# Artessay/RAGraph

Measured on AMD Instinct MI355X. Metric: retrieved-queries/sec (RAGraph_node forward: GCN encode + cosine/top-k retrieval + 3-hop propagate + decode), higher is better.
Workload: dtype f32 (exact results; candidates pre-filtered on bf16 / int8 MFMA with proven bounds)

## Files before the change

include/ragraph_hip.h:

```cpp
#ifndef RAGRAPH_HIP_H
#define RAGRAPH_HIP_H

#include <stddef.h>
#include <stdint.h>

#ifdef __cplusplus
extern "C" {
#endif

#define RAGRAPH_ABI_VERSION 1

#define RAGRAPH_OK 0
#define RAGRAPH_EINVAL (-1)
#define RAGRAPH_EUNSUPPORTED (-2)
#define RAGRAPH_EWORKSPACE (-3)
#define RAGRAPH_EDEVICE (-4)

#define RAGRAPH_ACT_NONE 0
#define RAGRAPH_ACT_RELU 1
#define RAGRAPH_ACT_PRELU 2
#define RAGRAPH_ACT_LEAKY 3
#define RAGRAPH_ACT_ELU 4

int ragraph_abi_version(void);
// ... 148 lines not shown
                               const int64_t* off, int64_t E, int64_t* out_col, int64_t* out_r, float* out_val,
                               void* stream);
int ragraph_spmm_csr_prelu_dev_f32(const int64_t* rowptr, const int32_t* col, const float* val, int64_t n, const float* X,
                                   int D, const float* bias, const float* alpha, float* Y, float* Z, int64_t nnz, void* ws,
                                   size_t ws_bytes, void* stream);
int ragraph_act_grad_prelu_dev_f32(const float* z, const float* gy, int64_t n, const float* alpha, float* gz,
                                   float* alpha_terms, void* stream);

size_t ragraph_radix_sort_workspace_bytes(int64_t n, int val_bytes);
int ragraph_radix_sort_u64(const uint64_t* keys_in, uint64_t* keys_out, const void* vals_in, void* vals_out, int val_bytes,
                           int64_t n, int bits, void* ws, size_t ws_bytes, void* stream);
size_t ragraph_scan_workspace_bytes(int64_t n);
int ragraph_scan_sum_i32(const int* in, int* out, int64_t n, int inclusive, void* ws, size_t ws_bytes, void* stream);

size_t ragraph_coo_to_csr_workspace_bytes(int64_t E, int64_t n);
int ragraph_coo_to_csr_i64(const int64_t* row, const int64_t* col, int64_t E, int64_t n, int sort_cols, int64_t* rowptr,
                           int64_t* perm, int32_t* out_col, void* ws, size_t ws_bytes, void* stream);
int ragraph_csr_row_ids_i64(const int64_t* rowptr, int64_t n, int64_t nnz, int64_t* rows, void* stream);

size_t ragraph_dense_to_csr_workspace_bytes(int64_t rows, int64_t cols);
int ragraph_dense_to_csr_f32(const float* a, int64_t rows, int64_t cols, int64_t lda, int64_t capacity, int64_t* rowptr,
                             int32_t* col, float* val, int64_t* status, void* ws, size_t ws_bytes, void* stream);

size_t ragraph_mask_positions_workspace_bytes(int64_t E);
int ragraph_mask_positions_i64(const unsigned char* mask, int64_t E, int64_t* pos, int64_t* count, void* ws, size_t ws_bytes,
                               void* stream);

int ragraph_spmm_csr_panels_f32(const int64_t* rowptr, const int32_t* col, const float* val, int64_t n, const float* X,
                                int64_t x_rows, int x_panels, int D, int act, float alpha, float* Y, int y_panels, void* stream);

int ragraph_spmm_linear_f32(const int64_t* rowptr, const int32_t* col, const float* val, int64_t M, const float* X, int K,
                            const float* W, int64_t N, const float* bias, int act, float alpha, float* Y, void* stream);

int ragraph_spmm_csr_tiled_f32(const int* wp, const int* col3, const float* val3, const unsigned short* row3, int RG, int C,
                               int64_t n, const float* X, int64_t x_rows, int x_panels, int D, int act, float alpha, float* Y,
                               int y_panels, void* stream);

int ragraph_csr_row_normalize_f32(const int64_t* rowptr, const float* val, int64_t n, float* val_out, void* stream);

int ragraph_segment_softmax_f32(const int64_t* rowptr, const float* x, int64_t n, float* out, void* stream);
int ragraph_segment_softmax_ws_f32(const int64_t* rowptr, const float* x, int64_t n, int64_t nnz, float* out, void* ws,
                                   size_t ws_bytes, void* stream);

int ragraph_axpby_f32(const float* a, float wa, const float* b, float wb, int64_t n, float* out, void* stream);

#define RAGRAPH_INTERP_MAX_TABLES 8
int ragraph_interp_normalize_f32(const float* const* tables, const float* weights, int S, int64_t n, int D, float* out,
                                 void* stream);

int ragraph_fuse_decode_f32(const float* query, const float* rag, int64_t n, int D, float wq, float wr, const float* W1,
                            const float* b1, int H, float slope, const float* W2, const float* b2, int C,
                            const float* rag_label, float lambda, float* out, void* stream);

int ragraph_softmax_mix_f32(const float* logits, const float* rag_label, int64_t B, int C, float lambda, int log_mode,
                            float* out, void* stream);

int ragraph_segment_reduce_f32(const float* X, int D, const int64_t* seg_ptr, int64_t G, const float* w, int mean_mode,
                               float* out, void* stream);

int ragraph_proto_cosine_f32(const float* emb, int64_t G, int D, const float* proto, int C, int mode, float* out,
                             void* stream);

int ragraph_sigmoid_gate_f32(const float* x, const float* z, int64_t n, float* out, void* stream);

int ragraph_time_rescale_f32(const int64_t* t, int64_t n, float t_min, float t_max, float* out, void* stream);

int ragraph_topk_rows_f32(const float* S, int64_t B, int64_t N, int64_t ld, int k, float* out_scores,
                          int64_t* out_idx, void* stream);

int ragraph_topk_select_rows_f32(const float* S, int64_t B, int64_t N, int64_t ld, int64_t k, float* out_kth,
                                 int64_t* out_idx, void* stream);
size_t ragraph_topk_select_rows_workspace_bytes(int64_t B, int64_t N);
int ragraph_topk_select_rows_ws_f32(const float* S, int64_t B, int64_t N, int64_t ld, int64_t k, float* out_kth,
                                    int64_t* out_idx, void* ws, size_t ws_bytes, void* stream);

#define RAGRAPH_TOPK_ORDERED_MAX 4096
size_t ragraph_topk_rows_large_workspace_bytes(int64_t B, int64_t N, int64_t k);
int ragraph_topk_rows_large_f32(const float* S, int64_t B, int64_t N, int64_t ld, int64_t k, float* out_scores,
                                int64_t* out_idx, void* ws, size_t ws_bytes, void* stream);

int ragraph_scatter_fill_f32(float* S, int64_t B, int64_t N, int64_t ld, const int64_t* rowptr, const int64_t* col,
                             float value, void* stream);

int ragraph_floyd_warshall_f32(const float* adj, int n, float* dist, void* stream);

int ragraph_position_code_f32(const float* dist, int n, const int64_t* anchors, int A, float dis_q, float* out,
                              void* stream);

int ragraph_position_codes_csr_f32(const int64_t* rowptr, const int32_t* col, const float* val, int64_t n,
                                   const int64_t* anchors, int A, float dis_q, float* codes, float* dist, void* stream);

#define RAGRAPH_POSITION_CODES_LONG_ROW 512
size_t ragraph_position_codes_csr_global_workspace_bytes(int64_t n, int A);
int ragraph_position_codes_csr_global_f32(const int64_t* rowptr, const int32_t* col, const float* val, int64_t n,
                                          const int64_t* anchors, int A, float dis_q, float* codes, float* dist, int rounds,
                                          int resume, int32_t* converged, void* ws, size_t ws_bytes, void* stream);

int ragraph_act_grad_f32(const float* y, const float* gy, int64_t n, int act, float alpha, float* gz, float* alpha_terms,
                         void* stream);
int ragraph_sigmoid_gate_grad_f32(const float* x, const float* z, const float* g, int64_t n, float* gx, float* gz, void* stream);
int ragraph_softmax_grad_f32(const float* p, const float* go, int64_t B, int C, float scale, float* out, void* stream);
int ragraph_mul_cols_f32(const float* x, const float* w, int64_t n, int D, float* out, void* stream);
int ragraph_mul_cols_act_f32(const float* x, const float* w, int64_t n, int D, int act, float alpha, float* out, void* stream);
int ragraph_mul_f32(const float* a, const float* b, int64_t n, float* out, void* stream);
int ragraph_proto_cosine_grad_f32(const float* emb, int64_t G, int D, const float* proto, int C, int mode, const float* out,
                                  const float* gout, float* gemb, void* stream);
// ... 79 lines not shown
```

ragraph_amd/RAGraph.py:

```python
import functools
import os

import torch
import torch.nn as nn

from . import autograd as A
from . import kernels as K
from .graph import as_csr
from .ragraph_utils import Propagation, TaskDecoder, ToyGraphBase


class RAGraph(nn.Module):

    flavour = "node"

    def __init__(self, pretrain_model, resource_dataset, feture_size, num_class, emb_size, finetune=True,
                 noise_finetune=False, device="cuda", build_rng="host") -> None:
        super().__init__()
        self.emb_size = emb_size
        self.num_class = num_class
        self.pretrain_model = pretrain_model
        self.retrieve_weight, self.label_weight, self.query_graph_hop = self._hyper()
        self.finetune = finetune
        self.noise_finetune = noise_finetune
# ... 9 lines not shown
            self.reset_parameters()
        self.to(device)

    def _hyper(self):
        return 0.5, 0.5, 3

    def reset_parameters(self):
        self.decoder.reset_parameters()

    def _queries(self, emb, g):
        return emb

    def _pool(self, x, g):
        return x

    query_shard = None

    def forward(self, features, adj, anchors=None):
        g = as_csr(adj)
        tgb = self.toy_graph_base
        mixed = getattr(tgb, "structure_weight", 0.0) != 0
        if mixed and (self.query_shard is not None or hasattr(tgb, "retrieve_reduced_rows")):
            raise K.RagraphNativeError("structure-aware retrieval (structure_weight != 0) runs on one GPU with the whole "
                                       "bank: the query-sharded and key-sharded forwards do not mix position codes")
        shards_queries = self.query_shard is not None and not self.training and self.flavour == "node"
        own_rows = not self.training and self.flavour == "node" and self._finishes_own_rows(tgb)
        if shards_queries:
            sliced = self._forward_sliced_encode(features, g, hybrid=own_rows)
            if sliced is not None:
                return sliced
        pretrain_embedddings = self.pretrain_model.inference(features, g)
        add_noise = self.training and self.noise_finetune
        if add_noise and getattr(tgb, "noise_rng", "host") != "device" and torch.cuda.is_current_stream_capturing():
            raise K.RagraphNativeError("noisy fine-tuning draws its noise on the host generator, as the reference does: "
                                       "its step cannot be captured in a HIP graph (train it eagerly, or set "
                                       "toy_graph_base.noise_rng = 'device')")
        queries = self._queries(pretrain_embedddings, g)
        pos = tgb.search_positions(g, None, anchors) if mixed else None
        if own_rows:
            return self._forward_key_shard(queries, pretrain_embedddings, g)
        if shards_queries:
            return self._forward_query_shard(queries, pretrain_embedddings, g)
        def hops():
            return self._pool(Propagation.aggregate_k_hop_features(g, pretrain_embedddings, self.query_graph_hop), g)

        join = None
        if (self.finetune and not (torch.is_grad_enabled() and pretrain_embedddings.requires_grad) and queries.is_cuda
                and queries.shape[0] >= self.OVERLAP_MIN_NODES):
            join = self._fork(hops, queries.device)
        if (join is not None and not add_noise and not torch.is_grad_enabled() and self.flavour == "node"
                and type(tgb).retrieve_reduced is ToyGraphBase.retrieve_reduced
                and os.environ.get("RAGRAPH_GATHER_MIX", "1") != "0"):
            _, idx = tgb.topk(queries, tgb.retrieve_num, pos) if mixed else tgb.topk(queries, tgb.retrieve_num)
            hidden, rag_label = K.gather_reduce_mix(tgb.resource_values, tgb.resource_labels, idx, join(),
                                                    1 - self.retrieve_weight, self.retrieve_weight)
            return A.softmax_mix(self.decoder(hidden), rag_label, self.label_weight)
        if add_noise:
            rag_embedding, rag_label = (tgb.retrieve_reduced_noisy(queries, search_positions=pos) if mixed
                                        else tgb.retrieve_reduced_noisy(queries))
        elif mixed:
            rag_embedding, rag_label, _ = tgb.retrieve_reduced(queries, search_positions=pos)
        else:
            rag_embedding, rag_label, _ = tgb.retrieve_reduced(queries)
        if not self.finetune:
            return rag_label
        query_embeddings = join() if join is not None else hops()
        return self._fuse_decode(query_embeddings, rag_embedding, rag_label)

    OVERLAP_MIN_NODES = 16384

    @staticmethod
    def _finishes_own_rows(tgb) -> bool:
        return (getattr(tgb, "values_replicated", False) and hasattr(tgb, "retrieve_reduced_rows")
                and (tgb.collective or tgb.emulate_world > 1))

    def _side_stream(self, device):
        st = getattr(self, "_side", None)
        if st is None or st.device != device:
            st = torch.cuda.Stream(device=device)
            self._side = st
        return st

    def _fork(self, fn, device):
        main = torch.cuda.current_stream()
        side = self._side_stream(device)
        side.wait_stream(main)
        with torch.cuda.stream(side):
            out = fn()

        def join():
            main.wait_stream(side)
            out.record_stream(main)
            return out
        return join

    def _fuse_decode(self, query_embeddings, rag_embedding, rag_label):
        fc1, fc2 = self.decoder.layers()
        trains = torch.is_grad_enabled() and (query_embeddings.requires_grad or rag_embedding.requires_grad or
                                              any(p.requires_grad for p in self.decoder.parameters()))
        if not trains and K.fuse_decode_fits(query_embeddings.shape[0], fc1.in_features, fc1.out_features, fc2.out_features):
            return K.fuse_decode(query_embeddings, rag_embedding, 1 - self.retrieve_weight, self.retrieve_weight,
                                 fc1.weight, fc1.bias, self.decoder.NEGATIVE_SLOPE, fc2.weight, fc2.bias, rag_label,
                                 self.label_weight)
        hidden = A.axpby(query_embeddings, 1 - self.retrieve_weight, rag_embedding, self.retrieve_weight)
        decode_label = self.decoder(hidden)
        return A.softmax_mix(decode_label, rag_label, self.label_weight)
# ... 79 lines not shown
```

ragraph_amd/_native.py:

```python
from __future__ import annotations

import ctypes
import os
import subprocess

import torch

_HERE = os.path.dirname(os.path.abspath(__file__))
CSRC = os.path.join(_HERE, "csrc")
SO_PATH = os.environ.get("RAGRAPH_HIP_SO", os.path.join(CSRC, "libragraph_hip.so"))

OK, EINVAL, EUNSUPPORTED, EWORKSPACE, EDEVICE = 0, -1, -2, -3, -4
ACT_NONE, ACT_RELU, ACT_PRELU, ACT_LEAKY, ACT_ELU = 0, 1, 2, 3, 4
TOPK_MAX = 64
TOPK_FILTER_MAX = 128
TOPK_ORDERED_MAX = 4096
TOPK_TAIL_MAX = 65536
LINEAR_GENERIC, LINEAR_SMALL, LINEAR_TILE, LINEAR_STREAM, LINEAR_NARROW = 0, 1, 2, 3, 4
INTERP_MAX_TABLES = 8
POSITION_CODES_LDS_MAX = 40000
POSITION_CODES_LONG_ROW = 512

_vp, _i64, _i32, _f32, _sz = ctypes.c_void_p, ctypes.c_int64, ctypes.c_int, ctypes.c_float, ctypes.c_size_t

# ... 49 lines not shown
    "ragraph_topk_cosine_mix_workspace_bytes": (_sz, [_i64, _i64, _i32, _i32, _i32]),
    "ragraph_topk_cosine_mix_f32": (_i32, [_vp, _i64, _vp, _i64, _i32, _vp, _vp, _i32, _f32, _f32, _i32, _i64, _vp, _vp, _vp,
                                          _sz, _vp]),
    "ragraph_topk_mix_rerank_workspace_bytes": (_sz, [_i64, _i32]),
    "ragraph_topk_mix_rerank_f32": (_i32, [_vp, _vp, _i64, _i32, _vp, _vp, _i64, _i32, _f32, _f32, _i32, _i64, _vp, _vp, _vp, _vp,
                                          _vp, _sz, _vp]),
    "ragraph_topk_rows_scatter_f32": (_i32, [_vp, _vp, _vp, _i64, _i32, _i64, _vp, _vp, _vp]),
    "ragraph_topk_merge_f32": (_i32, [_vp, _vp, _i32, _i64, _i32, _vp, _vp, _vp]),
    "ragraph_topk_cosine_tail_workspace_bytes": (_sz, [_i64, _i64, _i32, _i32]),
    "ragraph_topk_cosine_tail_f32": (_i32, [_vp, _i64, _vp, _i64, _i32, _i32, _i64, _vp, _vp, _vp, _vp, _vp, _sz, _vp]),
    "ragraph_topk_drop_rows_f32": (_i32, [_vp, _vp, _i64, _i32, _i64, _vp, _i64, _i32, _vp, _vp, _vp, _vp]),
    "ragraph_rows_retire_u32": (_i32, [_vp, _i64, _i64, _vp, _vp]),
    "ragraph_dedup_rows_workspace_bytes": (_sz, [_i64]),
    "ragraph_dedup_rows_f32": (_i32, [_vp, _i64, _i32, _vp, _vp, _vp, _vp, _vp, _sz, _vp]),
    "ragraph_topk_expand_groups_f32": (_i32, [_vp, _vp, _i32, _i64, _vp, _vp, _i64, _i64, _i32, _i64, _vp, _vp, _vp]),
    "ragraph_gather_rows_f32": (_i32, [_vp, _i64, _i32, _vp, _i64, _i64, _vp, _vp]),
    "ragraph_gather_reduce_f32": (_i32, [_vp, _i32, _vp, _i32, _i64, _vp, _i64, _i32, _i64, _f32, _vp, _vp, _vp]),
    "ragraph_gather_reduce_mix_f32": (_i32, [_vp, _i32, _vp, _i32, _i64, _vp, _i64, _i32, _i64, _f32, _vp, _f32, _f32, _vp, _vp, _vp]),
    "ragraph_linear_f32": (_i32, [_vp, _i64, _i32, _vp, _i64, _vp, _i32, _f32, _vp, _vp]),
    "ragraph_linear_plan": (_i32, [_i64, _i32, _i64, _i32, _i32, _vp]),
    "ragraph_linear_tn_workspace_bytes": (_sz, [_i64, _i32, _i32]),
    "ragraph_linear_tn_f32": (_i32, [_vp, _vp, _i64, _i32, _i32, _vp, _vp, _sz, _vp]),
    "ragraph_spmm_csr_f32": (_i32, [_vp, _vp, _vp, _i64, _vp, _i32, _vp, _i32, _f32, _f32, _vp, _vp, _vp]),
    "ragraph_radix_sort_workspace_bytes": (_sz, [_i64, _i32]),
    "ragraph_radix_sort_u64": (_i32, [_vp, _vp, _vp, _vp, _i32, _i64, _i32, _vp, _sz, _vp]),
    "ragraph_scan_workspace_bytes": (_sz, [_i64]),
    "ragraph_scan_sum_i32": (_i32, [_vp, _vp, _i64, _i32, _vp, _sz, _vp]),
    "ragraph_coo_to_csr_workspace_bytes": (_sz, [_i64, _i64]),
    "ragraph_coo_to_csr_i64": (_i32, [_vp, _vp, _i64, _i64, _i32, _vp, _vp, _vp, _vp, _sz, _vp]),
    "ragraph_csr_row_ids_i64": (_i32, [_vp, _i64, _i64, _vp, _vp]),
    "ragraph_dense_to_csr_workspace_bytes": (_sz, [_i64, _i64]),
    "ragraph_dense_to_csr_f32": (_i32, [_vp, _i64, _i64, _i64, _i64, _vp, _vp, _vp, _vp, _vp, _sz, _vp]),
    "ragraph_mask_positions_workspace_bytes": (_sz, [_i64]),
    "ragraph_mask_positions_i64": (_i32, [_vp, _i64, _vp, _vp, _vp, _sz, _vp]),
    "ragraph_spmm_csr_panels_f32": (_i32, [_vp, _vp, _vp, _i64, _vp, _i64, _i32, _i32, _i32, _f32, _vp, _i32, _vp]),
    "ragraph_spmm_linear_f32": (_i32, [_vp, _vp, _vp, _i64, _vp, _i32, _vp, _i64, _vp, _i32, _f32, _vp, _vp]),
    "ragraph_spmm_csr_tiled_f32": (_i32, [_vp, _vp, _vp, _vp, _i32, _i32, _i64, _vp, _i64, _i32, _i32, _i32, _f32, _vp, _i32, _vp]),
    "ragraph_csr_row_normalize_f32": (_i32, [_vp, _vp, _i64, _vp, _vp]),
    "ragraph_segment_softmax_f32": (_i32, [_vp, _vp, _i64, _vp, _vp]),
    "ragraph_segment_softmax_ws_f32": (_i32, [_vp, _vp, _i64, _i64, _vp, _vp, _sz, _vp]),
    "ragraph_sparse_workspace_bytes": (_sz, [_i64, _i32]),
    "ragraph_spmm_csr_ws_f32": (_i32, [_vp, _vp, _vp, _i64, _vp, _i32, _vp, _i32, _f32, _f32, _vp, _vp, _i64, _vp, _sz,
                                       _vp]),
    "ragraph_spmm_csr_rows_workspace_bytes": (_sz, [_i64, _i64, _i32]),
    "ragraph_spmm_csr_rows_f32": (_i32, [_vp, _vp, _vp, _i64, _vp, _i32, _vp, _i64, _vp, _i64, _vp, _sz, _vp]),
    "ragraph_csr_rows_offsets_workspace_bytes": (_sz, [_i64]),
    "ragraph_csr_rows_offsets_i64": (_i32, [_vp, _i64, _vp, _i64, _vp, _vp, _sz, _vp]),
    "ragraph_csr_rows_edges_f32": (_i32, [_vp, _vp, _vp, _vp, _i64, _vp, _i64, _vp, _vp, _vp, _vp]),
    "ragraph_axpby_f32": (_i32, [_vp, _f32, _vp, _f32, _i64, _vp, _vp]),
    "ragraph_interp_normalize_f32": (_i32, [_vp, _vp, _i32, _i64, _i32, _vp, _vp]),
    "ragraph_softmax_mix_f32": (_i32, [_vp, _vp, _i64, _i32, _f32, _i32, _vp, _vp]),
    "ragraph_fuse_decode_f32": (_i32, [_vp, _vp, _i64, _i32, _f32, _f32, _vp, _vp, _i32, _f32, _vp, _vp, _i32, _vp, _f32,
                                       _vp, _vp]),
    "ragraph_segment_reduce_f32": (_i32, [_vp, _i32, _vp, _i64, _vp, _i32, _vp, _vp]),
    "ragraph_proto_cosine_f32": (_i32, [_vp, _i64, _i32, _vp, _i32, _i32, _vp, _vp]),
    "ragraph_sigmoid_gate_f32": (_i32, [_vp, _vp, _i64, _vp, _vp]),
    "ragraph_time_rescale_f32": (_i32, [_vp, _i64, _f32, _f32, _vp, _vp]),
    "ragraph_topk_rows_f32": (_i32, [_vp, _i64, _i64, _i64, _i32, _vp, _vp, _vp]),
    "ragraph_topk_select_rows_f32": (_i32, [_vp, _i64, _i64, _i64, _i64, _vp, _vp, _vp]),
    "ragraph_topk_select_rows_workspace_bytes": (_sz, [_i64, _i64]),
    "ragraph_topk_select_rows_ws_f32": (_i32, [_vp, _i64, _i64, _i64, _i64, _vp, _vp, _vp, _sz, _vp]),
    "ragraph_topk_rows_large_workspace_bytes": (_sz, [_i64, _i64, _i64]),
    "ragraph_topk_rows_large_f32": (_i32, [_vp, _i64, _i64, _i64, _i64, _vp, _vp, _vp, _sz, _vp]),
    "ragraph_scatter_fill_f32": (_i32, [_vp, _i64, _i64, _i64, _vp, _vp, _f32, _vp]),
    "ragraph_floyd_warshall_f32": (_i32, [_vp, _i32, _vp, _vp]),
    "ragraph_position_code_f32": (_i32, [_vp, _i32, _vp, _i32, _f32, _vp, _vp]),
    "ragraph_position_codes_csr_f32": (_i32, [_vp, _vp, _vp, _i64, _vp, _i32, _f32, _vp, _vp, _vp]),
    "ragraph_position_codes_csr_global_workspace_bytes": (_sz, [_i64, _i32]),
    "ragraph_position_codes_csr_global_f32": (_i32, [_vp, _vp, _vp, _i64, _vp, _i32, _f32, _vp, _vp, _i32, _i32, _vp, _vp, _sz,
                                                     _vp]),
    "ragraph_act_grad_f32": (_i32, [_vp, _vp, _i64, _i32, _f32, _vp, _vp, _vp]),
    "ragraph_spmm_csr_prelu_dev_f32": (_i32, [_vp, _vp, _vp, _i64, _vp, _i32, _vp, _vp, _vp, _vp, _i64, _vp, _sz, _vp]),
    "ragraph_act_grad_prelu_dev_f32": (_i32, [_vp, _vp, _i64, _vp, _vp, _vp, _vp]),
    "ragraph_sigmoid_gate_grad_f32": (_i32, [_vp, _vp, _vp, _i64, _vp, _vp, _vp]),
    "ragraph_softmax_grad_f32": (_i32, [_vp, _vp, _i64, _i32, _f32, _vp, _vp]),
    "ragraph_mul_cols_f32": (_i32, [_vp, _vp, _i64, _i32, _vp, _vp]),
    "ragraph_mul_cols_act_f32": (_i32, [_vp, _vp, _i64, _i32, _i32, _f32, _vp, _vp]),
    "ragraph_mul_f32": (_i32, [_vp, _vp, _i64, _vp, _vp]),
    "ragraph_proto_cosine_grad_f32": (_i32, [_vp, _i64, _i32, _vp, _i32, _i32, _vp, _vp, _vp, _vp]),
    "ragraph_proto_cosine_grad_proto_workspace_bytes": (_sz, [_i64, _i32, _i32]),
    "ragraph_proto_cosine_grad_proto_f32": (_i32, [_vp, _i64, _i32, _vp, _i32, _i32, _vp, _vp, _vp, _vp, _sz, _vp]),
    "ragraph_axpby_dev_f32": (_i32, [_vp, _vp, _vp, _i32, _i32, _i64, _vp, _vp]),
    "ragraph_ingest_workspace_bytes": (_sz, [_i64, _i64]),
    "ragraph_csr_sym_normalized_f32": (_i32, [_vp, _vp, _i64, _i64, _vp, _vp, _vp, _vp, _vp, _sz, _vp]),
    "ragraph_binorm_edges_f32": (_i32, [_vp, _vp, _vp, _i64, _i64, _i64, _vp, _vp, _vp, _vp, _vp, _sz, _vp]),
    "ragraph_pagerank_workspace_bytes": (_sz, [_i64, _i64]),
    "ragraph_pagerank_f32": (_i32, [_vp, _vp, _vp, _vp, _vp, _vp, _i64, _i64, _f32, _f32, _i32, _vp, _vp, _vp, _sz, _vp]),
    "ragraph_sample_prob_f32": (_i32, [_vp, _vp, _vp, _i64, _f32, _f32, _vp, _vp]),
    "ragraph_csr_row_sums_f32": (_i32, [_vp, _vp, _i64, _vp, _vp]),
    "ragraph_position_codes_batch_f32": (_i32, [_vp, _i64, _i32, _vp, _i32, _f32, _vp, _vp, _vp]),
    "ragraph_topk_dot_masked_workspace_bytes": (_sz, [_i64, _i64, _i32, _i32, _i64]),
    "ragraph_topk_dot_masked_f32": (_i32, [_vp, _i64, _vp, _i64, _vp, _i64, _i32, _i32, _vp, _vp, _i64, _f32, _vp, _vp, _vp,
                                          _sz, _vp]),
    "ragraph_rank_metrics_workspace_bytes": (_sz, [_i64, _i32, _i64]),
    "ragraph_rank_metrics_f64": (_i32, [_vp, _i64, _i32, _vp, _vp, _vp, _i32, _i64, _vp, _vp, _sz, _vp]),
    "ragraph_lp_workspace_bytes": (_sz, []),
    "ragraph_lp_sample_i64": (_i32, [_vp, _vp, _i64, _i64, _i32, _vp, _vp, _vp, _sz, _vp]),
    "ragraph_lp_compare_loss_fwd_f32": (_i32, [_vp, _i64, _i32, _vp, _i32, _f32, _vp, _vp, _vp, _vp, _vp, _vp, _vp, _sz, _vp]),
    "ragraph_lp_combine_f32": (_i32, [_vp, _vp, _vp, _vp, _vp, _f32, _i64, _i32, _vp, _vp]),
    "ragraph_edge_hist_check_i64": (_i32, [_vp, _vp, _i64, _i64, _i64, _vp, _sz, _vp]),
    "ragraph_edge_neg_sample_i64": (_i32, [_vp, _vp, _i64, _i64, _vp, _i64, _i32, _i32, _vp, _vp, _vp, _sz, _vp]),
    "ragraph_noise_rows_i64": (_i32, [_vp, _vp, _i64, _i64, _i32, _i64, _vp, _i64, _vp]),
    "ragraph_gather_reduce_noisy_f32": (_i32, [_vp, _i32, _vp, _i32, _i64, _vp, _i64, _i32, _i64, _f32, _vp, _vp, _i64, _i32, _i64,
                                               _vp, _f32, _f32, _vp, _vp, _vp]),
    "ragraph_add_normal_noise_f32": (_i32, [_vp, _i64, _i64, _i32, _f32, _vp, _vp, _i64, _vp, _vp]),
    "ragraph_edge_rewrite_workspace_bytes": (_sz, [_i64]),
# ... 57 lines not shown
```

ragraph_amd/csrc/dense.hip:

```cpp
#include "common.h"

namespace ragraph {

constexpr int LBM = 64, LBN = 64, LKC = 32, LLD = LKC + 1;

__global__ void __launch_bounds__(256) linear_kernel(const float* __restrict__ X, int64_t M, int K,
                                                     const float* __restrict__ W, int64_t N,
                                                     const float* __restrict__ bias, int act, float alpha,
                                                     float* __restrict__ Y) {
  __shared__ float As[2][LBM * LLD];
  __shared__ float Bs[2][LBN * LLD];
  const int tid = threadIdx.x, lane = tid & 63, wave = tid >> 6;
  const int j = lane & 31, h = lane >> 5;
  const int wr = wave >> 1, wc = wave & 1;
  const int64_t m0 = (int64_t)blockIdx.x * LBM;
  const int64_t n0 = (int64_t)blockIdx.y * LBN;

  f32x16 acc;
#pragma unroll
  for (int r = 0; r < 16; ++r) acc[r] = 0.f;

  constexpr int PER = (LBM * LKC) / 256;
  float ra[2][PER], rb[2][PER];
  auto gload = [&](int k0, float (&pa)[PER], float (&pb)[PER]) {
#pragma unroll
    for (int u = 0; u < PER; ++u) {
      const int e = tid + u * 256;
      const int row = e / LKC, c = e % LKC;
      const int kk = k0 + c;
      const int64_t gm = m0 + row, gn = n0 + row;
      pa[u] = (gm < M && kk < K) ? X[gm * K + kk] : 0.f;
      pb[u] = (gn < N && kk < K) ? W[gn * K + kk] : 0.f;
    }
  };
  auto sstore = [&](int buf, const float (&pa)[PER], const float (&pb)[PER]) {
#pragma unroll
    for (int u = 0; u < PER; ++u) {
      const int e = tid + u * 256;
      const int row = e / LKC, c = e % LKC;
      As[buf][row * LLD + c] = pa[u];
      Bs[buf][row * LLD + c] = pb[u];
    }
  };
  auto compute = [&](int buf) {
    const float* a = As[buf] + (wr * 32 + j) * LLD + h;
    const float* b = Bs[buf] + (wc * 32 + j) * LLD + h;
#pragma unroll
    for (int kk = 0; kk < LKC / 2; ++kk) acc = __builtin_amdgcn_mfma_f32_32x32x2f32(a[2 * kk], b[2 * kk], acc, 0, 0, 0);
  };
  const int nch = (K + LKC - 1) / LKC;
  gload(0, ra[0], rb[0]);
  sstore(0, ra[0], rb[0]);
  if (nch > 1) gload(LKC, ra[1], rb[1]);
// ... 322 lines not shown
  for (int s = 0; s < nstages; ++s) {
    const bool more = s + 1 < nstages;
    stage_load(more ? s + 1 : s);
    __builtin_amdgcn_sched_barrier(0);
#pragma unroll 1
    for (int t = 0; t < C::TILES; ++t) {
      f32x16 acc;
#pragma unroll
      for (int r = 0; r < 16; ++r) acc[r] = 0.f;
      const float* arow = smem + (s & 1) * C::STAGE_FLOATS + (t * 32 + j) * C::ROW + h * (KD / 2);
#pragma unroll
      for (int c = 0; c < KD / 8; ++c) {
        const float4 v = *reinterpret_cast<const float4*>(arow + 4 * c);
        acc = __builtin_amdgcn_mfma_f32_32x32x2f32(v.x, breg[4 * c], acc, 0, 0, 0);
        acc = __builtin_amdgcn_mfma_f32_32x32x2f32(v.y, breg[4 * c + 1], acc, 0, 0, 0);
        acc = __builtin_amdgcn_mfma_f32_32x32x2f32(v.z, breg[4 * c + 2], acc, 0, 0, 0);
        acc = __builtin_amdgcn_mfma_f32_32x32x2f32(v.w, breg[4 * c + 3], acc, 0, 0, 0);
      }
      const int64_t m_base = (st0 + s) * C::STAGE_ROWS + t * 32 + 4 * h;
      if (n < N) {
#pragma unroll
        for (int r = 0; r < 16; ++r) {
          const int64_t m = m_base + (r & 3) + 8 * (r >> 2);
          if (m < M) {
            float v = acc[r];
            if (bias) v = __fadd_rn(v, bv);
            Y[m * N + n] = apply_act(v, act, alpha);
          }
        }
      }
    }
    if (more) stage_write((s + 1) & 1);
    __syncthreads();
  }
}

template <int KD>
struct AggLinCfg {
  static constexpr int THREADS = 1024, MFMA_THREADS = 512;
  static constexpr int LPR = KD / 4;
  static constexpr int GROUPS = (THREADS - MFMA_THREADS) / LPR;
  static constexpr int R = 2;
  static constexpr int STAGE_ROWS = R * GROUPS;
  static constexpr int TILES = STAGE_ROWS / 32;
  static constexpr int ROW = KD + 4;
  static constexpr int STAGE_FLOATS = STAGE_ROWS * ROW;
#ifndef RG_AGGLIN_NB
#define RG_AGGLIN_NB 4
#endif
  static constexpr int NB = RG_AGGLIN_NB;
  static constexpr size_t LDS_BYTES = sizeof(float) * NB * STAGE_FLOATS + sizeof(int) * 2 * NB;
};

__device__ __forceinline__ void agglin_wait(int* f, int target) {
#ifdef RG_AGGLIN_FREE_RUN
  return;
#endif
  int spins = 0;
  while (__hip_atomic_load(f, __ATOMIC_ACQUIRE, __HIP_MEMORY_SCOPE_WORKGROUP) < target) {
    __builtin_amdgcn_s_sleep(1);
    if (++spins > (1 << 26)) __builtin_trap();
  }
}
__device__ __forceinline__ void agglin_signal(int* f, int lane) {
  if (lane == 0) __hip_atomic_fetch_add(f, 1, __ATOMIC_RELEASE, __HIP_MEMORY_SCOPE_WORKGROUP);
}

template <int KD>
__global__ void __launch_bounds__(1024, 1) spmm_linear_stream_kernel(const int64_t* __restrict__ rowptr, const int32_t* __restrict__ col,
                                                                     const float* __restrict__ val, const float* __restrict__ X,
                                                                     int64_t M, const float* __restrict__ W, int64_t N,
                                                                     const float* __restrict__ bias, int act, float alpha,
                                                                     float* __restrict__ Y) {
  using C = AggLinCfg<KD>;
  extern __shared__ float4 lin_smem4[];
  float* smem = reinterpret_cast<float*>(lin_smem4);
  const int tid = threadIdx.x, lane = tid & 63, wave = __builtin_amdgcn_readfirstlane(tid >> 6);
  const int64_t total_stages = (M + C::STAGE_ROWS - 1) / C::STAGE_ROWS;
  const int64_t st0 = (int64_t)blockIdx.x * total_stages / gridDim.x;
  const int64_t st1 = (int64_t)(blockIdx.x + 1) * total_stages / gridDim.x;
  if (st0 >= st1) return;
  const int nstages = (int)(st1 - st0);
  int* ready = reinterpret_cast<int*>(smem + C::NB * C::STAGE_FLOATS);
  int* freed = ready + C::NB;
  if (tid < 2 * C::NB) ready[tid] = 0;
  __syncthreads();

  if (wave < 8) {
    const int j = lane & 31, h = lane >> 5;
    const int64_t n = (int64_t)blockIdx.y * 256 + wave * 32 + j;
    float breg[KD / 2];
    {
      const float4* wp = reinterpret_cast<const float4*>(W + (n < N ? n : N - 1) * KD);
#pragma unroll
      for (int c0 = 0; c0 < KD / 4; c0 += 16) {
#pragma unroll
        for (int c = c0; c < c0 + 16 && c < KD / 4; ++c) {
          const float4 v = wp[c];
          breg[2 * c] = h ? v.y : v.x;
          breg[2 * c + 1] = h ? v.w : v.z;
        }
#pragma unroll
        for (int c = c0; c < c0 + 16 && c < KD / 4; ++c) asm volatile("" : "+v"(breg[2 * c]), "+v"(breg[2 * c + 1]));
        asm volatile("" ::: "memory");
      }
    }
    const float bv = (bias && n < N) ? bias[n] : 0.f;
    for (int s = 0; s < nstages; ++s) {
      const int buf = s % C::NB;
      agglin_wait(ready + buf, 8 * (s / C::NB + 1));
#ifndef RG_AGGLIN_NO_MFMA
#pragma unroll 1
      for (int t = 0; t < C::TILES; ++t) {
        f32x16 acc;
#pragma unroll
        for (int r = 0; r < 16; ++r) acc[r] = 0.f;
        const float* arow = smem + buf * C::STAGE_FLOATS + (t * 32 + j) * C::ROW + h * (KD / 2);
#pragma unroll
        for (int c = 0; c < KD / 8; ++c) {
// ... 437 lines not shown
```

ragraph_amd/kernels.py:

```python
from __future__ import annotations

import collections
import ctypes
import os

import torch

from . import _native as N
from ._native import ACT_ELU, ACT_LEAKY, ACT_NONE, ACT_PRELU, ACT_RELU, RagraphNativeError
from ._native import LINEAR_GENERIC, LINEAR_NARROW, LINEAR_SMALL, LINEAR_STREAM, LINEAR_TILE
from .filter_stats import MAGIC_VALUE as FILTER_STATS_MAGIC, levels as filter_stats_levels, ord2f

_device_ok = False


def _ready():
    global _device_ok
    if not _device_ok:
        N.require_device()
        _device_ok = True
    return N.lib()


def _f32c(t: torch.Tensor, name: str) -> torch.Tensor:
# ... 929 lines not shown
        out = torch.empty_like(tables[0])
    elif (not isinstance(out, torch.Tensor) or out.dtype != torch.float32 or out.shape != tables[0].shape
          or out.device != tables[0].device or not out.is_contiguous()):
        raise RagraphNativeError("interp_normalize: out must be a contiguous fp32 tensor of the tables' shape and device")
    if n == 0:
        return out
    ptrs = (ctypes.c_void_p * len(tables))(*[t.data_ptr() for t in tables])
    ws = (ctypes.c_float * len(w))(*w)
    N.check(L.ragraph_interp_normalize_f32(ptrs, ws, len(tables), n, D, out.data_ptr(), _stream()), "interp_normalize")
    return out


def softmax_mix(logits: torch.Tensor, rag_label: torch.Tensor | None, lam: float = 0.0,
                log_mode: bool = False) -> torch.Tensor:
    L = _ready()
    logits = _f32c(logits, "softmax_mix.logits")
    lg = logits.reshape(-1, logits.shape[-1])
    rl = None if rag_label is None else _f32c(rag_label, "softmax_mix.rag_label").reshape(lg.shape)
    out = torch.empty_like(lg)
    N.check(L.ragraph_softmax_mix_f32(lg.data_ptr(), _ptr(rl), lg.shape[0], lg.shape[1], float(lam), int(log_mode),
                                      out.data_ptr(), _stream()), "softmax_mix")
    return out.reshape(logits.shape)


FUSE_DECODE_MAX_ROWS = 8192
FUSE_DECODE_LDS = 64 * 1024


def fuse_decode_fits(n: int, D: int, H: int, C: int) -> bool:
    return 0 < n <= FUSE_DECODE_MAX_ROWS and 4 * 4 * ((D + 3) // 4 * 4 + (H + 3) // 4 * 4 + C) <= FUSE_DECODE_LDS


def fuse_decode(query: torch.Tensor, rag: torch.Tensor, wq: float, wr: float, W1: torch.Tensor, b1: torch.Tensor | None,
                slope: float, W2: torch.Tensor, b2: torch.Tensor | None, rag_label: torch.Tensor | None,
                lam: float) -> torch.Tensor:
    L = _ready()
    query, rag = _f32c(query, "fuse_decode.query"), _f32c(rag, "fuse_decode.rag")
    W1, W2 = _f32c(W1, "fuse_decode.W1"), _f32c(W2, "fuse_decode.W2")
    b1 = None if b1 is None else _f32c(b1, "fuse_decode.b1")
    b2 = None if b2 is None else _f32c(b2, "fuse_decode.b2")
    n, D = query.shape
    H, C = W1.shape[0], W2.shape[0]
    if rag.shape != query.shape or W1.shape[1] != D or W2.shape[1] != H:
        raise ValueError(f"fuse_decode: shapes query {tuple(query.shape)} rag {tuple(rag.shape)} W1 {tuple(W1.shape)} "
                         f"W2 {tuple(W2.shape)}")
    rl = None if rag_label is None else _f32c(rag_label, "fuse_decode.rag_label").reshape(n, C)
    out = torch.empty((n, C), dtype=torch.float32, device=query.device)
    N.check(L.ragraph_fuse_decode_f32(query.data_ptr(), rag.data_ptr(), n, D, float(wq), float(wr), W1.data_ptr(),
                                      _ptr(b1), H, float(slope), W2.data_ptr(), _ptr(b2), C, _ptr(rl), float(lam),
                                      out.data_ptr(), _stream()), "fuse_decode")
    return out


def segment_reduce(x: torch.Tensor, seg_ptr: torch.Tensor, w: torch.Tensor | None = None,
                   mean_mode: bool = False) -> torch.Tensor:
    L = _ready()
    x = _f32c(x, "segment_reduce.x")
    seg_ptr = _idxc(seg_ptr, "segment_reduce.seg_ptr")
    wv = None if w is None else _f32c(w, "segment_reduce.w").reshape(-1)
    G = seg_ptr.numel() - 1
    out = torch.empty((G, x.shape[1]), dtype=torch.float32, device=x.device)
    N.check(L.ragraph_segment_reduce_f32(x.data_ptr(), x.shape[1], seg_ptr.data_ptr(), G, _ptr(wv), int(mean_mode),
                                         out.data_ptr(), _stream()), "segment_reduce")
    return out


def proto_cosine(emb: torch.Tensor, proto: torch.Tensor, mode: int = 0) -> torch.Tensor:
    L = _ready()
    emb = _f32c(emb, "proto_cosine.emb")
    proto = _f32c(proto, "proto_cosine.proto")
    G, D = emb.shape
    C = proto.shape[0]
    out = torch.empty((G, C), dtype=torch.float32, device=emb.device)
    N.check(L.ragraph_proto_cosine_f32(emb.data_ptr(), G, D, proto.data_ptr(), C, mode, out.data_ptr(), _stream()),
            "proto_cosine")
    return out


def proto_cosine_grad(emb: torch.Tensor, proto: torch.Tensor, mode: int, out: torch.Tensor, gout: torch.Tensor):
    L = _ready()
    emb, proto = _f32c(emb, "proto_cosine_grad.emb"), _f32c(proto, "proto_cosine_grad.proto")
    out, gout = _f32c(out, "proto_cosine_grad.out"), _f32c(gout, "proto_cosine_grad.gout")
    G, D = emb.shape
    gemb = torch.empty_like(emb)
    N.check(L.ragraph_proto_cosine_grad_f32(emb.data_ptr(), G, D, proto.data_ptr(), proto.shape[0], mode, out.data_ptr(),
                                            gout.data_ptr(), gemb.data_ptr(), _stream()), "proto_cosine_grad")
    return gemb


def proto_cosine_grad_proto(emb: torch.Tensor, proto: torch.Tensor, mode: int, out: torch.Tensor, gout: torch.Tensor):
    L = _ready()
    emb, proto = _f32c(emb, "proto_cosine_grad_proto.emb"), _f32c(proto, "proto_cosine_grad_proto.proto")
    out, gout = _f32c(out, "proto_cosine_grad_proto.out"), _f32c(gout, "proto_cosine_grad_proto.gout")
    G, D = emb.shape
    C = proto.shape[0]
    nbytes = int(L.ragraph_proto_cosine_grad_proto_workspace_bytes(G, C, D))
    ws = torch.empty(max(nbytes, 4), dtype=torch.uint8, device=emb.device)
    gproto = torch.empty_like(proto)
    N.check(L.ragraph_proto_cosine_grad_proto_f32(emb.data_ptr(), G, D, proto.data_ptr(), C, mode, out.data_ptr(), gout.data_ptr(),
                                                  gproto.data_ptr(), ws.data_ptr(), nbytes, _stream()), "proto_cosine_grad_proto")
    return gproto


def axpby_dev(a: torch.Tensor, b: torch.Tensor, w: torch.Tensor, ia: int, ib: int) -> torch.Tensor:
    L = _ready()
    a, b = _f32c(a, "axpby_dev.a"), _f32c(b, "axpby_dev.b")
# ... 783 lines not shown
```

Before: 5.817 million.

## Fuse gather-reduce-mix, MLP decode and softmax label mix into one warp-specialized kernel

Adds a single HIP kernel in which gather waves sum the top-k retrieved value and label rows and blend them with the propagated query embedding into an LDS stage ring. MFMA waves hold W1 in registers and compute the first decoder layer with LeakyReLU, then the second layer, the softmax and the label mix. This replaces the separate gather_reduce_mix launch, the decoder linear layers and the softmax_mix launch on the inference path, removing the global round trips for the hidden activations and logits. The trade-offs are a hand-synchronized producer/consumer ring with spin waits and support limited to D=H in {64,128,256}, C<=8 and k<=64.

Result: no change. 5.839 million (median of 6 runs) (+0.4%).

```diff
diff --git a/include/ragraph_hip.h b/include/ragraph_hip.h
--- a/include/ragraph_hip.h
+++ b/include/ragraph_hip.h
@@ -224,6 +224,10 @@
                             const float* b1, int H, float slope, const float* W2, const float* b2, int C,
                             const float* rag_label, float lambda, float* out, void* stream);
 
+int ragraph_gather_decode_mix_f32(const float* V, int D, const float* L, int C, int64_t N, const int64_t* idx, int64_t B,
+                                  int k, const float* A, float wa, float wb, const float* W1, const float* b1, int H,
+                                  float slope, const float* W2, const float* b2, float lambda, float* out, void* stream);
+
 int ragraph_softmax_mix_f32(const float* logits, const float* rag_label, int64_t B, int C, float lambda, int log_mode,
                             float* out, void* stream);
 
diff --git a/ragraph_amd/RAGraph.py b/ragraph_amd/RAGraph.py
--- a/ragraph_amd/RAGraph.py
+++ b/ragraph_amd/RAGraph.py
@@ -85,6 +85,13 @@
                 and type(tgb).retrieve_reduced is ToyGraphBase.retrieve_reduced
                 and os.environ.get("RAGRAPH_GATHER_MIX", "1") != "0"):
             _, idx = tgb.topk(queries, tgb.retrieve_num, pos) if mixed else tgb.topk(queries, tgb.retrieve_num)
+            fc1, fc2 = self.decoder.layers()
+            if (K.TAIL_ONE_LAUNCH and tgb.resource_labels is not None
+                    and K.gather_decode_fits(fc1.in_features, fc1.out_features, fc2.out_features, idx.shape[1])
+                    and tgb.resource_values.shape[1] == fc1.in_features):
+                return K.gather_decode_mix(tgb.resource_values, tgb.resource_labels, idx, join(), 1 - self.retrieve_weight,
+                                           self.retrieve_weight, fc1.weight, fc1.bias, self.decoder.NEGATIVE_SLOPE,
+                                           fc2.weight, fc2.bias, self.label_weight)
             hidden, rag_label = K.gather_reduce_mix(tgb.resource_values, tgb.resource_labels, idx, join(),
                                                     1 - self.retrieve_weight, self.retrieve_weight)
             return A.softmax_mix(self.decoder(hidden), rag_label, self.label_weight)
diff --git a/ragraph_amd/_native.py b/ragraph_amd/_native.py
--- a/ragraph_amd/_native.py
+++ b/ragraph_amd/_native.py
@@ -125,6 +125,8 @@
     "ragraph_softmax_mix_f32": (_i32, [_vp, _vp, _i64, _i32, _f32, _i32, _vp, _vp]),
     "ragraph_fuse_decode_f32": (_i32, [_vp, _vp, _i64, _i32, _f32, _f32, _vp, _vp, _i32, _f32, _vp, _vp, _i32, _vp, _f32,
                                        _vp, _vp]),
+    "ragraph_gather_decode_mix_f32": (_i32, [_vp, _i32, _vp, _i32, _i64, _vp, _i64, _i32, _vp, _f32, _f32, _vp, _vp, _i32, _f32,
+                                             _vp, _vp, _f32, _vp, _vp]),
     "ragraph_segment_reduce_f32": (_i32, [_vp, _i32, _vp, _i64, _vp, _i32, _vp, _vp]),
     "ragraph_proto_cosine_f32": (_i32, [_vp, _i64, _i32, _vp, _i32, _i32, _vp, _vp]),
     "ragraph_sigmoid_gate_f32": (_i32, [_vp, _vp, _i64, _vp, _vp]),
diff --git a/ragraph_amd/csrc/dense.hip b/ragraph_amd/csrc/dense.hip
--- a/ragraph_amd/csrc/dense.hip
+++ b/ragraph_amd/csrc/dense.hip
@@ -1,4 +1,5 @@
 #include "common.h"
+#include "stage_ring.h"
 
 namespace ragraph {
 
@@ -427,19 +428,6 @@
   static constexpr size_t LDS_BYTES = sizeof(float) * NB * STAGE_FLOATS + sizeof(int) * 2 * NB;
 };
 
-__device__ __forceinline__ void agglin_wait(int* f, int target) {
-#ifdef RG_AGGLIN_FREE_RUN
-  return;
-#endif
-  int spins = 0;
-  while (__hip_atomic_load(f, __ATOMIC_ACQUIRE, __HIP_MEMORY_SCOPE_WORKGROUP) < target) {
-    __builtin_amdgcn_s_sleep(1);
-    if (++spins > (1 << 26)) __builtin_trap();
-  }
-}
-__device__ __forceinline__ void agglin_signal(int* f, int lane) {
-  if (lane == 0) __hip_atomic_fetch_add(f, 1, __ATOMIC_RELEASE, __HIP_MEMORY_SCOPE_WORKGROUP);
-}
 
 template <int KD>
 __global__ void __launch_bounds__(1024, 1) spmm_linear_stream_kernel(const int64_t* __restrict__ rowptr, const int32_t* __restrict__ col,
diff --git a/ragraph_amd/csrc/stage_ring.h b/ragraph_amd/csrc/stage_ring.h
--- /dev/null
+++ b/ragraph_amd/csrc/stage_ring.h
@@ -0,0 +1,20 @@
+#pragma once
+#include "common.h"
+
+namespace ragraph {
+
+__device__ __forceinline__ void agglin_wait(int* f, int target) {
+#ifdef RG_AGGLIN_FREE_RUN
+  return;
+#endif
+  int spins = 0;
+  while (__hip_atomic_load(f, __ATOMIC_ACQUIRE, __HIP_MEMORY_SCOPE_WORKGROUP) < target) {
+    __builtin_amdgcn_s_sleep(1);
+    if (++spins > (1 << 26)) __builtin_trap();
+  }
+}
+__device__ __forceinline__ void agglin_signal(int* f, int lane) {
+  if (lane == 0) __hip_atomic_fetch_add(f, 1, __ATOMIC_RELEASE, __HIP_MEMORY_SCOPE_WORKGROUP);
+}
+
+}
diff --git a/ragraph_amd/csrc/tail.hip b/ragraph_amd/csrc/tail.hip
--- /dev/null
+++ b/ragraph_amd/csrc/tail.hip
@@ -0,0 +1,308 @@
+#include "common.h"
+#include "stage_ring.h"
+
+namespace ragraph {
+
+constexpr int TAIL_MAX_C = 8;
+
+template <int KD>
+struct TailCfg {
+  static constexpr int THREADS = 768, MFMA_THREADS = 512;
+  static constexpr int MFMA_WAVES = KD / 32;
+  static constexpr int GATHER_WAVES = 4;
+  static constexpr int STAGE_ROWS = 32;
+  static constexpr int RPW = STAGE_ROWS / GATHER_WAVES;
+  static constexpr int ROW = KD + 4;
+  static constexpr int STAGE_FLOATS = STAGE_ROWS * ROW;
+  static constexpr int NB = 3;
+  static constexpr int H1_OFF = NB * STAGE_FLOATS;
+  static constexpr int W2_OFF = H1_OFF + STAGE_FLOATS;
+  static constexpr int LAB_OFF = W2_OFF + TAIL_MAX_C * ROW;
+  static constexpr int LG_OFF = LAB_OFF + NB * STAGE_ROWS * TAIL_MAX_C;
+  static constexpr int CNT_OFF = LG_OFF + STAGE_ROWS * TAIL_MAX_C;
+  static constexpr int NCNT = 2 * NB + 2;
+  static constexpr size_t LDS_BYTES = sizeof(float) * CNT_OFF + sizeof(int) * NCNT;
+};
+
+template <int KD>
+__global__ void __launch_bounds__(768, 1) gather_decode_mix_kernel(const float* __restrict__ V, const float* __restrict__ L, int C,
+                                                                   int64_t N, const int64_t* __restrict__ idx, int64_t B, int k,
+                                                                   const float* __restrict__ A, float wa, float wb,
+                                                                   const float* __restrict__ W1, const float* __restrict__ b1,
+                                                                   float slope, const float* __restrict__ W2,
+                                                                   const float* __restrict__ b2, float lambda,
+                                                                   float* __restrict__ out) {
+  using Cf = TailCfg<KD>;
+  extern __shared__ float4 tail_smem4[];
+  float* smem = reinterpret_cast<float*>(tail_smem4);
+  const int tid = threadIdx.x, lane = tid & 63, wave = __builtin_amdgcn_readfirstlane(tid >> 6);
+  const int64_t total_stages = (B + Cf::STAGE_ROWS - 1) / Cf::STAGE_ROWS;
+  const int64_t st0 = (int64_t)blockIdx.x * total_stages / gridDim.x;
+  const int64_t st1 = (int64_t)(blockIdx.x + 1) * total_stages / gridDim.x;
+  if (st0 >= st1) return;
+  const int nstages = (int)(st1 - st0);
+  float* h1 = smem + Cf::H1_OFF;
+  float* W2s = smem + Cf::W2_OFF;
+  float* lab = smem + Cf::LAB_OFF;
+  int* ready = reinterpret_cast<int*>(smem + Cf::CNT_OFF);
+  int* freed = ready + Cf::NB;
+  int* h1_ready = freed + Cf::NB;
+  int* h1_done = h1_ready + 1;
+  if (tid < Cf::NCNT) ready[tid] = 0;
+  for (int e = tid; e < KD * TAIL_MAX_C; e += Cf::THREADS) {
+    const int c = e / KD, kk = e % KD;
+    W2s[c * Cf::ROW + kk] = c < C ? W2[e] : 0.f;
+  }
+  __syncthreads();
+
+  if (wave < 8) {
+    constexpr int NW = Cf::MFMA_WAVES;
+    if (wave >= NW) return;
+    const int j = lane & 31, h = lane >> 5;
+    const int n = wave * 32 + j;
+    float breg[KD / 2];
+    {
+      const float4* wp = reinterpret_cast<const float4*>(W1 + (int64_t)n * KD);
+      auto chunk = [&](const int c0, const int w) __attribute__((always_inline)) {
+#pragma unroll
+        for (int c = c0; c < c0 + w; ++c) {
+          const float4 v = wp[c];
+          breg[2 * c] = h ? v.y : v.x;
+          breg[2 * c + 1] = h ? v.w : v.z;
+        }
+#pragma unroll
+        for (int c = c0; c < c0 + w; ++c) asm volatile("" : "+v"(breg[2 * c]), "+v"(breg[2 * c + 1]));
+        asm volatile("" ::: "memory");
+      };
+      if constexpr (KD == 256) {
+        chunk(0, 16); chunk(16, 16); chunk(32, 8); chunk(40, 8); chunk(48, 8); chunk(56, 4); chunk(60, 4);
+      } else {
+#pragma unroll
+        for (int c0 = 0; c0 < KD / 4; c0 += 16) chunk(c0, 16);
+      }
+    }
+    const float bv = b1 ? b1[n] : 0.f;
+    for (int s = 0; s < nstages; ++s) {
+      const int buf = s % Cf::NB;
+      agglin_wait(ready + buf, Cf::GATHER_WAVES * (s / Cf::NB + 1));
+#ifndef RG_TAIL_NO_MFMA
+      f32x16 acc;
+#pragma unroll
+      for (int r = 0; r < 16; ++r) acc[r] = 0.f;
+      const float* arow = smem + buf * Cf::STAGE_FLOATS + j * Cf::ROW + h * (KD / 2);
+#pragma unroll
+      for (int c = 0; c < KD / 8; ++c) {
+        const float4 v = *reinterpret_cast<const float4*>(arow + 4 * c);
+        acc = __builtin_amdgcn_mfma_f32_32x32x2f32(v.x, breg[4 * c], acc, 0, 0, 0);
+        acc = __builtin_amdgcn_mfma_f32_32x32x2f32(v.y, breg[4 * c + 1], acc, 0, 0, 0);
+        acc = __builtin_amdgcn_mfma_f32_32x32x2f32(v.z, breg[4 * c + 2], acc, 0, 0, 0);
+        acc = __builtin_amdgcn_mfma_f32_32x32x2f32(v.w, breg[4 * c + 3], acc, 0, 0, 0);
+      }
+      agglin_signal(freed + buf, lane);
+      if (s > 0) agglin_wait(h1_done, NW * s);
+#pragma unroll
+      for (int r = 0; r < 16; ++r) {
+        float v = acc[r];
+        if (b1) v = __fadd_rn(v, bv);
+        h1[((r & 3) + 8 * (r >> 2) + 4 * h) * Cf::ROW + n] = apply_act(v, RAGRAPH_ACT_LEAKY, slope);
+      }
+      agglin_signal(h1_ready, lane);
+      {
+        agglin_wait(h1_ready, NW * (s + 1));
+        int ln = lane;
+        asm volatile("" : "+v"(ln));
+        float lam = lambda;
+        asm volatile("" : "+s"(lam));
+        constexpr int RPD = Cf::STAGE_ROWS / NW;
+        const int cq = ln & 7;
+        float* lg = smem + Cf::LG_OFF;
+        for (int rr = ln >> 3; rr < RPD; rr += 8) {
+          const int row = wave * RPD + rr;
+          const float4* xr = reinterpret_cast<const float4*>(h1 + row * Cf::ROW);
+          const float4* wr = reinterpret_cast<const float4*>(W2s + cq * Cf::ROW);
+          float a = 0.f;
+#pragma unroll 4
+          for (int k4 = 0; k4 < KD / 4; ++k4) {
+            const float4 x = xr[k4], w = wr[k4];
+            a = fmaf(x.x, w.x, a); a = fmaf(x.y, w.y, a); a = fmaf(x.z, w.z, a); a = fmaf(x.w, w.w, a);
+          }
+          if (b2 && cq < C) a = __fadd_rn(a, b2[cq]);
+          lg[row * TAIL_MAX_C + cq] = a;
+        }
+        __builtin_amdgcn_fence(__ATOMIC_RELEASE, "wavefront");
+        __builtin_amdgcn_wave_barrier();
+        __builtin_amdgcn_fence(__ATOMIC_ACQUIRE, "wavefront");
+        const int row = wave * RPD + ln;
+        const int64_t m_row = (st0 + s) * Cf::STAGE_ROWS + row;
+        if (ln < RPD && m_row < B) {
+          const float one_m = 1.f - lam;
+          const float* x = lg + row * TAIL_MAX_C;
+          const float* rl = lab + (buf * Cf::STAGE_ROWS + row) * TAIL_MAX_C;
+          float mx = x[0];
+#pragma clang loop vectorize(disable) interleave(disable) unroll(disable)
+          for (int c = 1; c < C; ++c) mx = fmaxf(mx, x[c]);
+          float sb = 0.f;
+#pragma clang loop vectorize(disable) interleave(disable) unroll(disable)
+          for (int c = 0; c < C; ++c) sb = __fadd_rn(sb, expf(x[c] - mx));
+          const float sum = __fadd_rn(0.f, sb);
+#pragma clang loop vectorize(disable) interleave(disable) unroll(disable)
+          for (int c = 0; c < C; ++c) {
+            float p = expf(x[c] - mx) / sum;
+            p = __fadd_rn(__fmul_rn(p, one_m), __fmul_rn(rl[c], lam));
+            out[m_row * C + c] = p;
+          }
+        }
+        agglin_signal(h1_done, lane);
+      }
+#else
+      agglin_signal(freed + buf, lane);
+      agglin_signal(h1_done, lane);
+#endif
+    }
+    return;
+  }
+
+  __builtin_amdgcn_s_setprio(3);
+  constexpr int D4 = KD / 4;
+  const int g = wave - 8;
+  const bool colok = lane < D4;
+  const int cc = colok ? lane : 0;
+  const int lc = lane < C ? lane : 0;
+  const float4* V4 = reinterpret_cast<const float4*>(V);
+  const float4* A4 = reinterpret_cast<const float4*>(A);
+  auto row_of = [&](int64_t mine, int u) {
+    return ((int64_t)__builtin_amdgcn_readlane((int)(mine >> 32), u) << 32) | (unsigned)__builtin_amdgcn_readlane((int)mine, u);
+  };
+  auto load_idx = [&](int stage, int i) {
+    const int64_t b = (st0 + stage) * Cf::STAGE_ROWS + g * Cf::RPW + i;
+    int64_t r = -1;
+    if (stage < nstages && b < B && lane < k) {
+      r = idx[b * k + lane];
+      if (r < 0 || r >= N) r = -1;
+    }
+    return r;
+  };
+  constexpr int GS = 10;
+  int64_t mA = load_idx(0, 0), mB = load_idx(0, 1);
+#ifdef RG_TAIL_NO_GATHER
+  const int kg = 0;
+#else
+  const int kg = k;
+#endif
+#pragma unroll 1
+  for (int stage = 0; stage < nstages; ++stage) {
+    const int buf = stage % Cf::NB;
+#pragma unroll
+    for (int p = 0; p < Cf::RPW / 2; ++p) {
+      const int rowA = g * Cf::RPW + 2 * p;
+      const int64_t bA = (st0 + stage) * Cf::STAGE_ROWS + rowA, bB = bA + 1;
+      const int64_t nA = load_idx(p + 1 < Cf::RPW / 2 ? stage : stage + 1, (2 * p + 2) % Cf::RPW);
+      const int64_t nB = load_idx(p + 1 < Cf::RPW / 2 ? stage : stage + 1, (2 * p + 3) % Cf::RPW);
+      const float4 hA = A4[(bA < B ? bA : B - 1) * D4 + cc], hB = A4[(bB < B ? bB : B - 1) * D4 + cc];
+      float4 sA = make_float4(0.f, 0.f, 0.f, 0.f), sB = sA;
+      float tA = 0.f, tB = 0.f;
+      for (int j0 = 0; j0 < kg; j0 += GS) {
+        float4 va[GS], vb[GS];
+        float la[GS], lb[GS];
+        bool oka[GS], okb[GS];
+#pragma unroll
+        for (int u = 0; u < GS; ++u) {
+          const int64_t r = j0 + u < kg ? row_of(mA, j0 + u) : -1;
+          oka[u] = r >= 0;
+          va[u] = V4[(oka[u] ? r : 0) * D4 + cc];
+          la[u] = L[(oka[u] ? r : 0) * C + lc];
+        }
+#pragma unroll
+        for (int u = 0; u < GS; ++u) {
+          const int64_t r = j0 + u < kg ? row_of(mB, j0 + u) : -1;
+          okb[u] = r >= 0;
+          vb[u] = V4[(okb[u] ? r : 0) * D4 + cc];
+          lb[u] = L[(okb[u] ? r : 0) * C + lc];
+        }
+#pragma unroll
+        for (int u = 0; u < GS; ++u) {
+          if (j0 + u < kg) {
+            const float4 x = oka[u] ? va[u] : make_float4(0.f, 0.f, 0.f, 0.f);
+            sA.x = __fadd_rn(sA.x, x.x); sA.y = __fadd_rn(sA.y, x.y); sA.z = __fadd_rn(sA.z, x.z); sA.w = __fadd_rn(sA.w, x.w);
+            if (oka[u]) tA = __fadd_rn(tA, la[u]);
+          }
+        }
+#pragma unroll
+        for (int u = 0; u < GS; ++u) {
+          if (j0 + u < kg) {
+            const float4 x = okb[u] ? vb[u] : make_float4(0.f, 0.f, 0.f, 0.f);
+            sB.x = __fadd_rn(sB.x, x.x); sB.y = __fadd_rn(sB.y, x.y); sB.z = __fadd_rn(sB.z, x.z); sB.w = __fadd_rn(sB.w, x.w);
+            if (okb[u]) tB = __fadd_rn(tB, lb[u]);
+          }
+        }
+      }
+      sA.x = __fadd_rn(__fmul_rn(hA.x, wa), __fmul_rn(sA.x, wb)); sA.y = __fadd_rn(__fmul_rn(hA.y, wa), __fmul_rn(sA.y, wb));
+      sA.z = __fadd_rn(__fmul_rn(hA.z, wa), __fmul_rn(sA.z, wb)); sA.w = __fadd_rn(__fmul_rn(hA.w, wa), __fmul_rn(sA.w, wb));
+      sB.x = __fadd_rn(__fmul_rn(hB.x, wa), __fmul_rn(sB.x, wb)); sB.y = __fadd_rn(__fmul_rn(hB.y, wa), __fmul_rn(sB.y, wb));
+      sB.z = __fadd_rn(__fmul_rn(hB.z, wa), __fmul_rn(sB.z, wb)); sB.w = __fadd_rn(__fmul_rn(hB.w, wa), __fmul_rn(sB.w, wb));
+      if (p == 0 && stage >= Cf::NB) {
+        agglin_wait(freed + buf, Cf::MFMA_WAVES * (stage / Cf::NB));
+        agglin_wait(h1_done, Cf::MFMA_WAVES * (stage - Cf::NB + 1));
+      }
+      if (colok) {
+        float* d = smem + buf * Cf::STAGE_FLOATS + rowA * Cf::ROW + 2 * lane;
+        d[0] = sA.x; d[1] = sA.z;
+        d[KD / 2] = sA.y; d[KD / 2 + 1] = sA.w;
+        d += Cf::ROW;
+        d[0] = sB.x; d[1] = sB.z;
+        d[KD / 2] = sB.y; d[KD / 2 + 1] = sB.w;
+      }
+      if (lane < TAIL_MAX_C) {
+        float* lw = lab + (buf * Cf::STAGE_ROWS + rowA) * TAIL_MAX_C + lane;
+        lw[0] = lane < C ? tA / (float)k : 0.f;
+        lw[TAIL_MAX_C] = lane < C ? tB / (float)k : 0.f;
+      }
+      mA = nA;
+      mB = nB;
+    }
+    agglin_signal(ready + buf, lane);
+  }
+}
+
+template <int KD>
+static int launch_gather_decode_mix(const float* V, const float* L, int C, int64_t N, const int64_t* idx, int64_t B, int k,
+                                    const float* A, float wa, float wb, const float* W1, const float* b1, float slope,
+                                    const float* W2, const float* b2, float lambda, float* out, hipStream_t st) {
+  using Cf = TailCfg<KD>;
+  static DeviceOnce lds_once;
+  if (hipError_t e = raise_dynamic_lds(lds_once, &gather_decode_mix_kernel<KD>, (int)Cf::LDS_BYTES); e != hipSuccess) {
+    set_error("gather_decode_mix: cannot raise dynamic LDS limit: %s", hipGetErrorString(e));
+    return RAGRAPH_EDEVICE;
+  }
+  const int64_t total_stages = cdiv(B, Cf::STAGE_ROWS);
+  int64_t wgs = device_cus_multiple_of_8();
+  if (wgs > total_stages) wgs = total_stages;
+  hipLaunchKernelGGL(gather_decode_mix_kernel<KD>, dim3((unsigned)wgs), dim3(Cf::THREADS), Cf::LDS_BYTES, st, V, L, C, N, idx, B, k,
+                     A, wa, wb, W1, b1, slope, W2, b2, lambda, out);
+  RG_CHECK_LAUNCH("gather_decode_mix");
+  return RAGRAPH_OK;
+}
+
+}
+
+using namespace ragraph;
+
+extern "C" int ragraph_gather_decode_mix_f32(const float* V, int D, const float* L, int C, int64_t N, const int64_t* idx,
+                                             int64_t B, int k, const float* A, float wa, float wb, const float* W1,
+                                             const float* b1, int H, float slope, const float* W2, const float* b2,
+                                             float lambda, float* out, void* stream) {
+  RG_REQUIRE(V && L && idx && A && W1 && W2 && out, RAGRAPH_EINVAL, "gather_decode_mix: null pointer");
+  RG_REQUIRE(D == 64 || D == 128 || D == 256, RAGRAPH_EUNSUPPORTED, "gather_decode_mix: D=%d not in {64, 128, 256}", D);
+  RG_REQUIRE(H == D, RAGRAPH_EUNSUPPORTED, "gather_decode_mix: H=%d must equal D=%d", H, D);
+  RG_REQUIRE(C >= 1 && C <= TAIL_MAX_C, RAGRAPH_EUNSUPPORTED, "gather_decode_mix: C=%d not in [1,%d]", C, TAIL_MAX_C);
+  RG_REQUIRE(k >= 1 && k <= 64, RAGRAPH_EUNSUPPORTED, "gather_decode_mix: k=%d not in [1,64]", k);
+  RG_REQUIRE(N >= 1 && B >= 0, RAGRAPH_EINVAL, "gather_decode_mix: bad shape");
+  RG_REQUIRE(aligned16(V) && aligned16(A) && aligned16(W1), RAGRAPH_EINVAL, "gather_decode_mix: V, A, W1 must be 16-B aligned");
+  if (B == 0) return RAGRAPH_OK;
+  hipStream_t st = as_stream(stream);
+  switch (D) {
+    case 64: return launch_gather_decode_mix<64>(V, L, C, N, idx, B, k, A, wa, wb, W1, b1, slope, W2, b2, lambda, out, st);
+    case 128: return launch_gather_decode_mix<128>(V, L, C, N, idx, B, k, A, wa, wb, W1, b1, slope, W2, b2, lambda, out, st);
+    default: return launch_gather_decode_mix<256>(V, L, C, N, idx, B, k, A, wa, wb, W1, b1, slope, W2, b2, lambda, out, st);
+  }
+}
diff --git a/ragraph_amd/kernels.py b/ragraph_amd/kernels.py
--- a/ragraph_amd/kernels.py
+++ b/ragraph_amd/kernels.py
@@ -1005,6 +1005,40 @@
     return out
 
 
+TAIL_ONE_LAUNCH = os.environ.get("RAGRAPH_TAIL_ONE_LAUNCH", "1") != "0"
+GATHER_DECODE_MAX_C = 8
+GATHER_DECODE_MAX_K = 64
+
+
+def gather_decode_fits(D: int, H: int, C: int, k: int, idx_base: int = 0, inference: bool = True) -> bool:
+    return (inference and idx_base == 0 and D in (64, 128, 256) and H == D and 1 <= C <= GATHER_DECODE_MAX_C
+            and 1 <= k <= GATHER_DECODE_MAX_K)
+
+
+def gather_decode_mix(v: torch.Tensor, labels: torch.Tensor, idx: torch.Tensor, a: torch.Tensor, wa: float, wb: float,
+                      W1: torch.Tensor, b1: torch.Tensor | None, slope: float, W2: torch.Tensor, b2: torch.Tensor | None,
+                      lam: float) -> torch.Tensor:
+    L = _ready()
+    v, labels = _f32c(v, "gather_decode_mix.v"), _f32c(labels, "gather_decode_mix.labels")
+    idx = _idxc(idx, "gather_decode_mix.idx")
+    a = _f32c(a, "gather_decode_mix.a")
+    W1, W2 = _f32c(W1, "gather_decode_mix.W1"), _f32c(W2, "gather_decode_mix.W2")
+    b1 = None if b1 is None else _f32c(b1, "gather_decode_mix.b1")
+    b2 = None if b2 is None else _f32c(b2, "gather_decode_mix.b2")
+    B, k = idx.shape
+    n, D = v.shape
+    H, C = W1.shape[0], W2.shape[0]
+    if (tuple(a.shape) != (B, D) or tuple(labels.shape) != (n, C) or W1.shape[1] != D or W2.shape[1] != H
+            or (b1 is not None and b1.numel() != H) or (b2 is not None and b2.numel() != C)):
+        raise RagraphNativeError(f"gather_decode_mix: shapes v {tuple(v.shape)} labels {tuple(labels.shape)} idx {tuple(idx.shape)} "
+                                 f"a {tuple(a.shape)} W1 {tuple(W1.shape)} W2 {tuple(W2.shape)}")
+    out = torch.empty((B, C), dtype=torch.float32, device=v.device)
+    N.check(L.ragraph_gather_decode_mix_f32(v.data_ptr(), D, labels.data_ptr(), C, n, idx.data_ptr(), B, k, a.data_ptr(), float(wa),
+                                            float(wb), W1.data_ptr(), _ptr(b1), H, float(slope), W2.data_ptr(), _ptr(b2),
+                                            float(lam), out.data_ptr(), _stream()), "gather_decode_mix")
+    return out
+
+
 def segment_reduce(x: torch.Tensor, seg_ptr: torch.Tensor, w: torch.Tensor | None = None,
                    mean_mode: bool = False) -> torch.Tensor:
     L = _ready()
```
